# oppo-us-research/PoP-Net

Measured on AMD Instinct MI355X. Metric: depth-frames/sec end-to-end (480x640), higher is better.
Workload: dtype bf16

## Files before the change

popnet_amd/csrc/api.hip:

```cpp
#pragma clang fp contract(off)
#include <cmath>
#include <cstdio>
#include <cstdlib>
#include <cstring>
#include "pn_internal.h"
#include "preproc_pixel.h"

template <typename TIN>
__global__ void preprocess_kernel(const TIN *__restrict__ depth, float *__restrict__ out, int B, int H, int W, int S,
                                  double scale_x, double scale_y, float dmax, float mean, float stdv) {
    const unsigned pix = blockIdx.x * blockDim.x + threadIdx.x;
    if (pix >= (unsigned)(S * S)) return;
    const int b = blockIdx.y;
    const int dy = (int)(pix / (unsigned)S);
    const int dx = (int)(pix - (unsigned)dy * (unsigned)S);
    const size_t gid = (size_t)b * S * S + pix;

    out[gid] = pn_preproc_pixel(depth + (size_t)b * H * W, H, W, dy, dx, scale_x, scale_y, dmax, mean, stdv);
}

PnSwitches pn_read_switches() {
    auto set = [](const char *name) { return getenv(name) != nullptr; };
    auto num = [](const char *name, int unset) { const char *e = getenv(name); return e ? atoi(e) : unset; };
    auto is = [](const char *name, const char *value) { const char *e = getenv(name); return e && !strcmp(e, value); };
    PnSwitches s;
    s.no_conv3 = set("POPNET_NO_CONV3");
    s.conv3_rpg8 = set("POPNET_CONV3_RPG8");
    s.conv3_pt14 = num("POPNET_CONV3_PT14", 0);
    s.conv3_nbuf2 = set("POPNET_CONV3_NBUF2");
    s.generic_c64_off = num("POPNET_GENERIC_C64", 1) == 0;
    if (set("POPNET_CONV4")) s.conv4 = num("POPNET_CONV4", 0) == 0 ? 0 : 1;
    s.no_mix = set("POPNET_NO_MIX");
    s.no_bblock = set("POPNET_NO_BBLOCK");
    s.bblock_x3 = num("POPNET_BBLOCK_X3", 0) != 0;
    s.bb64_static = set("POPNET_BB64_STATIC");
    s.bb64_halves = num("POPNET_BB64_HALVES", 1) == 2 ? 2 : 1;
    s.no_tailfuse = set("POPNET_NO_TAILFUSE");
    s.no_poolfuse = set("POPNET_NO_POOLFUSE");
    s.no_stempool = set("POPNET_NO_STEMPOOL");
    s.no_embed3 = set("POPNET_NO_EMBED3");
    s.train_x3_wide = set("POPNET_TRAIN_X3_WIDE");
    s.train_wgrad_novec = set("POPNET_TRAIN_WGRAD_NOVEC");
    s.trainx_one_stream = num("POPNET_TRAINX_STREAMS", 0) == 1;
    s.trainx_stem_handover = set("POPNET_TRAINX_STEM_HANDOVER");
    s.trainx_stem_gather = is("POPNET_TRAINX_STEM_FWD", "gather");
    s.trainx_stem_bn_separate = is("POPNET_TRAINX_STEM_BN", "separate");
    s.trainx_stem_depth = num("POPNET_TRAINX_STEM_DEPTH", 2);
    s.trainx_pack_gather = is("POPNET_TRAINX_PACK", "gather");
    s.trainx_legacy_wgrad = is("POPNET_TRAINX_WGRAD", "legacy");
    return s;
}

extern "C" {

int pn_abi_version(void) { return PN_ABI_VERSION; }
int pn_build_experiments(void) { return 0; }

pn_ctx *pn_create(int device_id) {
    pn_ctx *ctx = new pn_ctx();
    ctx->device = device_id;
    int ndev = 0;
    hipError_t e = hipGetDeviceCount(&ndev);
    if (e != hipSuccess || device_id < 0 || device_id >= ndev) {
        char buf[256];
        snprintf(buf, sizeof buf, "pn_create: device %d not available (%d devices, %s)", device_id, ndev,
                 hipGetErrorString(e));
        ctx->err = buf;
        ctx->device = -1;
        return ctx;
    }
    hipDeviceProp_t prop;
    if (hipGetDeviceProperties(&prop, device_id) == hipSuccess) ctx->num_cus = prop.multiProcessorCount;
    return ctx;
}

void pn_destroy(pn_ctx *ctx) {
    if (!ctx) return;
    if (ctx->parse_ws) (void)hipFree(ctx->parse_ws);
    pn_parse_big_free(ctx);
    if (ctx->train_ws) (void)hipFree(ctx->train_ws);
    for (void *p : ctx->train_ws_retired) (void)hipFree(p);
    for (auto &e : ctx->train_packs) (void)hipFree(e.buf);
    if (ctx->train_pack_table) (void)hipFree(ctx->train_pack_table);
    delete ctx;
}

int pn_last_error(pn_ctx *ctx, char *buf, size_t buf_len) {
    if (!ctx) return 0;
    if (buf && buf_len) {
        size_t n = ctx->err.size() < buf_len - 1 ? ctx->err.size() : buf_len - 1;
        memcpy(buf, ctx->err.data(), n);
        buf[n] = 0;
    }
    return (int)ctx->err.size();
}

int pn_preprocess(pn_ctx *ctx, const void *depth_dev, int depth_dtype, int B, int H, int W, float *out_dev, int S,
                  float depth_max, float depth_mean, float depth_std, void *hip_stream) {
    if (!ctx) return PN_ERR_INVALID;
    if (ctx->device < 0) return pn_set_error(ctx, PN_ERR_STATE, "context has no device");
    if (!depth_dev || !out_dev || B < 1 || H < 2 || W < 2 || S < 1)
        return pn_set_error(ctx, PN_ERR_INVALID, "pn_preprocess: bad arguments");
    if (W == 2 * S && H == 2 * S)
        return pn_set_error(ctx, PN_ERR_UNSUPPORTED, "pn_preprocess: %dx%d -> %d is an exact 2x decimation, where cv2.resize(INTER_LINEAR) runs INTER_AREA instead: not built", W, H, S);
    const double inv_x = (double)S / (double)W, inv_y = (double)S / (double)H;
    const double scale_x = 1.0 / inv_x, scale_y = 1.0 / inv_y;
    if (B > 65535 || (size_t)S * S > 0x7fffffffu) return pn_set_error(ctx, PN_ERR_INVALID, "pn_preprocess: batch or output size out of range");
    dim3 grid((unsigned)(((size_t)S * S + 255) / 256), (unsigned)B), block(256);
    hipStream_t s = (hipStream_t)hip_stream;
    if (depth_dtype == PN_DEPTH_F16)
        hipLaunchKernelGGL(preprocess_kernel<_Float16>, grid, block, 0, s, (const _Float16 *)depth_dev, out_dev, B, H, W, S,
                           scale_x, scale_y, depth_max, depth_mean, depth_std);
    else if (depth_dtype == PN_DEPTH_F32)
        hipLaunchKernelGGL(preprocess_kernel<float>, grid, block, 0, s, (const float *)depth_dev, out_dev, B, H, W, S,
// ... 26 lines not shown
```

popnet_amd/csrc/conv4_kernel.h:

```cpp
#pragma once
#include "conv3_kernel.h"

#define PN4_ASLOT 8192
constexpr int PN4_RING = 3;
constexpr int PN4_PITCH = 32;
#define PN4_ARING (PN4_RING * PN4_ASLOT)
#define PN4_BQUART (5 * PN4_PITCH * 32 + 1024)
#define PN4_BSTRIP (2 * PN4_BQUART)
#define PN4_BBUF (2 * PN4_BSTRIP)
#define PN4_LDS (PN4_ARING + 2 * PN4_BBUF)

__device__ __forceinline__ void conv4_body(const ConvProblem &P, const int block_x) {
    typedef __bf16 T;
    constexpr int KS = 3, KK = 9, PT = 7, CT = 4, PITCH = PN4_PITCH;
    extern __shared__ __attribute__((aligned(16))) char smem[];

    if (block_x >= P.nblocks) return;
    int bx;
    {
        const int nb = P.nblocks, xcd = block_x & 7, idx = block_x >> 3;
        const int qq = nb >> 3, rr = nb & 7;
        bx = (xcd < rr ? xcd * (qq + 1) : rr * (qq + 1) + (xcd - rr) * qq) + idx;
    }
    const int tid = threadIdx.x;
    const int lane = tid & 63;
    const int wave = __builtin_amdgcn_readfirstlane(tid >> 6);
    const int wp = wave >> 1, wc = wave & 1;
    const int c = lane & 15, q = lane >> 4;

    const int cb = bx % P.cout_blocks;
    const int pair = bx / P.cout_blocks;
    const int nstrips = P.B * P.tiles_per_img;
    const int sid_raw = pair * 2 + wp;
    const bool strip_ok = sid_raw < nstrips;
    const int sid = strip_ok ? sid_raw : nstrips - 1;
    const int tile = sid % P.tiles_per_img;
    const int b = sid / P.tiles_per_img;
    const int ty = tile / P.tiles_x, tx = tile - ty * P.tiles_x;
    const int oy0 = ty * P.R, ox0 = tx * P.Wt;
    const int R = min(P.R, P.Ho - oy0);
    const int Wo = P.Wo;
    const int Wc = min(P.Wt, Wo - ox0);
    const int npix = R * Wc;
    const int HC = Wc + KS - 1;
    const int iy0 = oy0 - 1, ix0 = ox0 - 1;
    const float inv_wc = 1.0f / (float)Wc;
    const int nchunks = P.cin_chunks;

    const char *aptr = (const char *)P.wpack + ((size_t)cb * (size_t)(P.ksteps + 3) * 8 + 2 * wave) * 1024;
    const unsigned alane16 = (unsigned)lane * 16u;
    auto dma_a = [&](int slot) {
        const unsigned dst = (unsigned)(slot * PN4_ASLOT) + (unsigned)__builtin_amdgcn_readfirstlane(wave * 2048);
        pn_glds16_s<0>(aptr, alane16, dst);
        pn_glds16_s<0>(aptr + 1024, alane16, dst + 1024u);
        aptr += PN4_ASLOT;
    };

    const size_t frame_b = ((size_t)b * P.H * P.W * P.in_cs + P.in_coff) * 2;
    const char *img = (const char *)P.in + frame_b;
    const unsigned zero_rel = P.in_zero_off - (unsigned)frame_b;
    unsigned boff[6];
#pragma unroll
    for (int j = 0; j < 6; ++j) {
        const int px = lane >> 1;
        const int iy = iy0 + j, ix = ix0 + px;
        const bool inb = px < HC && (unsigned)ix < (unsigned)P.W && (unsigned)iy < (unsigned)P.H;
        boff[j] = inb ? (unsigned)((iy * P.W + ix) * P.in_cs * 2 + wc * 32 + (lane & 1) * 16) : zero_rel;
    }
    const int nhalves = nchunks * 2, wrap_h = P.in_wrap * 2;
    auto dma_b = [&](int j, int buf, int hh) {
        const unsigned dst = (unsigned)(PN4_ARING + buf * PN4_BBUF + j * (PITCH * 32)) +
                             (unsigned)__builtin_amdgcn_readfirstlane(wp * PN4_BSTRIP + wc * PN4_BQUART);
        const int hs = hh < nhalves ? (hh >= wrap_h ? hh - wrap_h : hh) : 0;
        pn_glds16_s<0>(img + (size_t)hs * 64, boff[j], dst);
    };

#pragma unroll
    for (int j = 0; j < 6; ++j) dma_b(j, 0, 0);
    dma_a(0); dma_a(1); dma_a(2);

    int baddr[PT];
#pragma unroll
    for (int pt = 0; pt < PT; ++pt) {
        const int slot = pt * 16 + c;
        const int s = slot < npix ? slot : 0;
        const int ry = (int)(((float)s + 0.5f) * inv_wc);
        const int rx = s - ry * Wc;
        baddr[pt] = PN4_ARING + wp * PN4_BSTRIP + (q >> 1) * PN4_BQUART + (q & 1) * 16 + (ry * PITCH + rx) * 32;
    }
    const int aaddr = wc * 4096 + lane * 16;
    f32x4 acc[CT][PT];
#pragma unroll
    for (int ct = 0; ct < CT; ++ct)
#pragma unroll
        for (int pt = 0; pt < PT; ++pt) acc[ct][pt] = f32x4{0.f, 0.f, 0.f, 0.f};

    const bool active = (cb * 2 + wc) * 64 < P.cout;

    asm volatile("s_waitcnt vmcnt(0)\n\ts_barrier" ::: "memory");

#define PN4_BOFF(j) (((((j) / PT) / KK) & 1) * PN4_BBUF + (((((j) / PT) % KK) / KS) * PITCH + ((((j) / PT) % KK) % KS)) * 32)
    constexpr int BQ = 6;
    static_assert((2 * KK * PT) % BQ == 0, "queue slot of an item must not depend on the chunk");
    bf16x8 aq[2][CT], bq[BQ];
    if (active) {
#pragma unroll
        for (int ct = 0; ct < CT; ++ct) aq[0][ct] = *reinterpret_cast<const bf16x8 *>(smem + aaddr + ct * 1024);
#pragma unroll
        for (int j = 0; j < BQ - 1; ++j) bq[j] = *reinterpret_cast<const bf16x8 *>(smem + baddr[j % PT] + PN4_BOFF(j));
    }
    asm volatile("s_waitcnt lgkmcnt(0)\n\ts_barrier" ::: "memory");

    auto kloop = [&](auto mathc) {
        constexpr bool MATH = decltype(mathc)::value;
        for (int chunk = 0; chunk < nchunks; ++chunk) {
#pragma clang loop unroll(full)
            for (int ph = 0; ph < 2 * KK; ++ph) {
                const int tap = ph % KK, half = ph / KK;
                const int hh = chunk * 2 + half;
                const int anext = aaddr + ((ph + 1) % 3) * PN4_ASLOT;
                if (tap < 6) dma_b(tap, (half + 1) & 1, hh + 1);
                dma_a(ph % 3);
                if (MATH) {
                    __builtin_amdgcn_sched_barrier(0);
#pragma clang loop unroll(full)
                    for (int pt = 0; pt < PT; ++pt) {
                        const int j = ph * PT + pt, jr = j + BQ - 1;
                        if (pt < CT)
                            aq[(ph + 1) & 1][pt] = *reinterpret_cast<const bf16x8 *>(smem + anext + pt * 1024);
                        bq[jr % BQ] = *reinterpret_cast<const bf16x8 *>(smem + baddr[jr % PT] + PN4_BOFF(jr % (2 * KK * PT)));
#pragma unroll
                        for (int ct = 0; ct < CT; ++ct)
                            acc[ct][pt] = __builtin_amdgcn_mfma_f32_16x16x32_bf16(aq[ph & 1][ct], bq[j % BQ], acc[ct][pt], 0, 0, 0);
                        if (pt < CT) __builtin_amdgcn_sched_group_barrier(0x100, 2, 0);
                        else __builtin_amdgcn_sched_group_barrier(0x100, 1, 0);
                        __builtin_amdgcn_sched_group_barrier(0x008, CT, 0);
                    }
                    __builtin_amdgcn_sched_barrier(0);
                }
                if (tap < 6) asm volatile("s_waitcnt vmcnt(3) lgkmcnt(0)\n\ts_barrier" ::: "memory");
                else asm volatile("s_waitcnt vmcnt(2) lgkmcnt(0)\n\ts_barrier" ::: "memory");
            }
        }
    };
    if (active) kloop(std::true_type{});
    else kloop(std::false_type{});
#undef PN4_BOFF
    asm volatile("s_waitcnt vmcnt(0)" ::: "memory");
    if (!active || !strip_ok) return;

    constexpr int LC = CT * 4;
    const int wave_c0 = (cb * 2 + wc) * 64;
    const int cw = wave_c0 + LC * q;
    const int cout = P.cout, act = P.act;
    float bias[LC];
#pragma unroll
    for (int ct = 0; ct < CT; ++ct) {
        const f32x4 b4 = *reinterpret_cast<const PN_GLOBAL f32x4 *>((const PN_GLOBAL float *)P.bias + cw + 4 * ct);
        bias[4 * ct + 0] = b4[0]; bias[4 * ct + 1] = b4[1]; bias[4 * ct + 2] = b4[2]; bias[4 * ct + 3] = b4[3];
    }
    const int res_cs = P.res_cs, out_cs = P.out_cs, Ho = P.Ho;
    const int split = P.split, res_split = P.res_split;
    const unsigned pix0 = (unsigned)((b * Ho + oy0) * Wo + ox0);
    const bool full = wave_c0 + 64 <= cout && P.out && !P.out_nchw;
    if (full) {
        PN_GLOBAL T *ob = (PN_GLOBAL T *)P.out + P.out_coff + cw;
        const PN_GLOBAL T *rb = P.res ? (const PN_GLOBAL T *)P.res + P.res_coff + cw : nullptr;
        auto finish = [&](auto actc, auto resc) {
            constexpr int ACT = decltype(actc)::value;
            constexpr bool RES = decltype(resc)::value;
#pragma clang loop unroll(full)
            for (int pt = 0; pt < PT; ++pt) {
                const int slot = pt * 16 + c;
                const unsigned t = (unsigned)(baddr[pt] - PN4_ARING - wp * PN4_BSTRIP - (q >> 1) * PN4_BQUART) >> 5;
                const unsigned opix = PITCH == 32 ? pix0 + (t >> 5) * (unsigned)Wo + (t & 31u) : pix0 + (t / (unsigned)PITCH) * (unsigned)Wo + (t % (unsigned)PITCH);
                float v[LC];
#pragma unroll
                for (int ct = 0; ct < CT; ++ct)
#pragma unroll
                    for (int i = 0; i < 4; ++i) v[4 * ct + i] = acc[ct][pt][i] + bias[4 * ct + i];
                if (RES) {
                    for (int pl = 0; pl < (res_split ? 2 : 1); ++pl) {
                        T rv[LC];
                        const PN_GLOBAL u32x4 *rp = reinterpret_cast<const PN_GLOBAL u32x4 *>(rb + (opix * (unsigned)res_cs + (unsigned)(pl * res_split)));
                        reinterpret_cast<u32x4 *>(rv)[0] = rp[0];
                        reinterpret_cast<u32x4 *>(rv)[1] = rp[1];
#pragma unroll
                        for (int k = 0; k < LC; ++k) v[k] += (float)rv[k];
                    }
                }
#pragma unroll
                for (int k = 0; k < LC; ++k) {
                    if (ACT == PN_ACT_RELU) v[k] = v[k] > 0.f ? v[k] : 0.f;
                    else if (ACT == PN_ACT_LEAKY) v[k] = v[k] > 0.f ? v[k] : v[k] * 0.1f;
                    else if (ACT != PN_ACT_NONE) v[k] = pn_activate(v[k], act, cw + k, P.yolo_naf);
                }
                for (int pl = 0; pl < (split ? 2 : 1); ++pl) {
                    T ov[LC];
#pragma unroll
                    for (int k = 0; k < LC; ++k) {
                        const T hi = (T)v[k];
                        ov[k] = pl == 1 ? (T)(v[k] - (float)hi) : hi;
                    }
                    if (slot < npix) {
                        PN_GLOBAL u32x4 *op = reinterpret_cast<PN_GLOBAL u32x4 *>(ob + (opix * (unsigned)out_cs + (unsigned)(pl * split)));
                        op[0] = reinterpret_cast<u32x4 *>(ov)[0];
                        op[1] = reinterpret_cast<u32x4 *>(ov)[1];
                    }
                }
            }
        };
        if (P.res) {
            if (act == PN_ACT_RELU) finish(std::integral_constant<int, PN_ACT_RELU>{}, std::true_type{});
            else if (act == PN_ACT_LEAKY) finish(std::integral_constant<int, PN_ACT_LEAKY>{}, std::true_type{});
            else if (act == PN_ACT_NONE) finish(std::integral_constant<int, PN_ACT_NONE>{}, std::true_type{});
            else finish(std::integral_constant<int, -1>{}, std::true_type{});
        } else {
            if (act == PN_ACT_RELU) finish(std::integral_constant<int, PN_ACT_RELU>{}, std::false_type{});
            else if (act == PN_ACT_LEAKY) finish(std::integral_constant<int, PN_ACT_LEAKY>{}, std::false_type{});
            else if (act == PN_ACT_NONE) finish(std::integral_constant<int, PN_ACT_NONE>{}, std::false_type{});
            else finish(std::integral_constant<int, -1>{}, std::false_type{});
        }
        return;
    }
    {
        const PN_GLOBAL T *res_base = P.res ? (const PN_GLOBAL T *)P.res + P.res_coff + cw : nullptr;
        PN_GLOBAL T *out_base = P.out ? (PN_GLOBAL T *)P.out + P.out_coff + cw : nullptr;
        PN_GLOBAL float *nchw = (PN_GLOBAL float *)P.out_nchw;
#pragma clang loop unroll(full)
        for (int pt = 0; pt < PT; ++pt) {
            const int slot = pt * 16 + c;
            if (slot >= npix || cw >= cout) continue;
            const int ry = (int)(((float)slot + 0.5f) * inv_wc);
            const int rx = slot - ry * Wc;
            const unsigned opix = pix0 + (unsigned)(ry * Wo + rx);
#pragma unroll
            for (int ct = 0; ct < CT; ++ct)
#pragma unroll
                for (int i = 0; i < 4; ++i) {
                    const int k = 4 * ct + i;
                    if (cw + k >= cout) continue;
                    float v = acc[ct][pt][i] + bias[k];
                    if (res_base) v += (float)res_base[opix * (unsigned)res_cs + k];
                    if (res_base && res_split) v += (float)res_base[opix * (unsigned)res_cs + res_split + k];
                    v = pn_activate(v, act, cw + k, P.yolo_naf);
                    if (out_base) {
                        const T hi = (T)v;
                        out_base[opix * (unsigned)out_cs + k] = hi;
                        if (split) {
                            out_base[opix * (unsigned)out_cs + split + k] = (T)(v - (float)hi);
                        }
                    }
                    if (nchw) nchw[((size_t)b * cout + cw + k) * ((size_t)Ho * Wo) + (size_t)(oy0 + ry) * Wo + (ox0 + rx)] = v;
                }
        }
    }
}

__global__ __launch_bounds__(256, 2) void conv4_kernel(const ConvProblem *__restrict__ probs) {
    conv4_body(probs[blockIdx.y], (int)blockIdx.x);
}

static int conv4_launch(pn_ctx *ctx, const ConvLaunch &L, hipStream_t stream) {
    const size_t lds = PN4_LDS;
    static PnLdsAttr attr;
    if (int rc = pn_lds_attr(ctx, attr, reinterpret_cast<const void *>(conv4_kernel), lds)) return rc;
    hipLaunchKernelGGL(conv4_kernel, dim3(L.max_blocks, L.nprob), dim3(256), lds, stream, L.probs_dev);
    PN_HIP_CHECK(ctx, hipGetLastError());
    return PN_OK;
}
```

popnet_amd/csrc/net.hip:

```cpp
#include <cmath>
#include <cstdarg>
#include <cstdio>
#include <algorithm>
#include <cstdlib>
#include <cstring>
#include <map>
#include <memory>
#include <vector>
#include "pn_internal.h"
#include "conv_plan.h"
#include "preproc_pixel.h"

namespace {

struct HostTensor {
    std::vector<int64_t> shape;
    std::vector<float> data;
    size_t numel() const { return data.size(); }
};

struct Buf {
    void *p = nullptr;
    int H = 0, W = 0, C = 0;
    int plane = 0;
// ... 692 lines not shown
    int A1 = new_buf(n, H2, W2, 64);
    int X0 = new_buf(n, H4, W4, 64), X1 = new_buf(n, H4, W4, 64), XT = new_buf(n, H4, W4, 64);
    int Y0 = new_buf(n, H8, W8, 128), Y1 = new_buf(n, H8, W8, 128), YT = new_buf(n, H8, W8, 128), YD = new_buf(n, H8, W8, 128);
    int Na = new_buf(n, H8, W8, 256), Nb = new_buf(n, H8, W8, 256);
    int Ha = new_buf(n, H16, W16, 256), Hb = new_buf(n, H16, W16, 256), Hc = new_buf(n, H16, W16, 128);

    if (int rc = add_stem(n, A1)) return rc;
    std::vector<std::vector<int>> levels;
    auto level = [&](std::vector<int> ids) { levels.push_back(ids); };
    if (n->prec == PN_PREC_BF16 && !n->x3 && n->input_dim == 1 && !n->sw.no_stempool) n->steps.back().stem_pool_buf = X0;
    else levels.push_back({-1, 1, A1, X0, 64, 0});
    int cur = X0, other = X1;
    for (int i = 0; i < 3; ++i) {
        std::string p = "model0.layer1." + std::to_string(i);
        level({add_conv(n, p + ".conv1", p + ".bn1", 3, 1, cur, 0, XT, 0, PN_ACT_RELU)});
        level({add_conv(n, p + ".conv2", p + ".bn2", 3, 1, XT, 0, other, 0, PN_ACT_RELU, cur)});
        std::swap(cur, other);
    }
    {
        const bool embed = n->prec == PN_PREC_BF16 && !n->sw.no_embed3;
        const int c1 = add_conv(n, "model0.layer2.0.conv1", "model0.layer2.0.bn1", 3, 2, cur, 0, YT, 0, PN_ACT_RELU);
        const int cd = add_conv(n, "model0.layer2.0.downsample.0", "model0.layer2.0.downsample.1", embed ? 3 : 1, 2, cur, 0, YD, 0, PN_ACT_NONE);
        n->convs[cd].embed3 = embed;
        level({c1, cd});
    }
    level({add_conv(n, "model0.layer2.0.conv2", "model0.layer2.0.bn2", 3, 1, YT, 0, Y0, 0, PN_ACT_RELU, YD)});
    int yc = Y0, yo = Y1;
    for (int i = 1; i < 4; ++i) {
        std::string p = "model0.layer2." + std::to_string(i);
        level({add_conv(n, p + ".conv1", p + ".bn1", 3, 1, yc, 0, YT, 0, PN_ACT_RELU)});
        level({add_conv(n, p + ".conv2", p + ".bn2", 3, 1, YT, 0, yo, 0, PN_ACT_RELU, yc)});
        std::swap(yc, yo);
    }
    n->named["feat"] = {yc, {0, 128}};
    level({add_conv(n, "model1.0", "model1.1", 3, 1, yc, 0, Na, 0, PN_ACT_LEAKY)});
    level({add_conv(n, "model1.3", "model1.4", 3, 1, Na, 0, Nb, 0, PN_ACT_LEAKY)});
    level({add_conv(n, "model1.6", "model1.7", 3, 1, Nb, 0, Na, 0, PN_ACT_LEAKY)});
    level({add_conv(n, "model1.9", "model1.10", 3, 1, Na, 0, Nb, 0, PN_ACT_LEAKY)});
    level({add_conv(n, "model1.12", "", 3, 1, Nb, 0, Na, 0, PN_ACT_NONE)});
    level({add_conv(n, "model2_1.0", "model2_1.1", 3, 1, Na, 0, Nb, 0, PN_ACT_LEAKY)});
    levels.push_back({-1, 2, Nb, Ha, 256, 0});
    level({add_conv(n, "model2_2.0", "model2_2.1", 3, 1, Ha, 0, Hb, 0, PN_ACT_LEAKY)});
    level({add_conv(n, "model2_3.0", "model2_3.1", 3, 1, Hb, 0, Hc, 0, PN_ACT_LEAKY)});
    level({add_conv(n, "model2_4.0", "", 3, 1, Hc, 0, -1, 0, PN_ACT_YOLO, -1, 3)});

    for (auto &cs : n->convs)
        if (int rc = prepare_conv(n, cs)) return rc;
    for (auto &cs : n->convs) n->flops_per_frame += cs.flops;
    fuse_basic_blocks(n, levels);
    for (auto &lv : levels) {
        if (lv[0] == -1) add_pool(n, lv[1], lv[2], lv[3], lv[4], lv[5]);
        else if (lv[0] == -2) { if (int rc = add_bblock(n, lv[1], lv[2])) return rc; }
        else add_conv_level(n, lv);
    }
    return PN_OK;
}

int refresh_problems(pn_net *n, int B, hipStream_t stream) {
    for (auto &st : n->steps) {
        if (st.type != Step::CONV) continue;
        const ConvSpec &c0 = n->convs[st.conv_ids[0]];
        const int BC = c0.kern == 4 ? 128 : (c0.kern == 3 ? c0.wc * 32 : pn_cfg_couts(c0.cfg));
        st.host_probs.clear();
        int max_blocks = 0;
        bool two_bufs = false, has_tail = false, pool_tail = false;
        for (int id : st.conv_ids) {
            const ConvSpec &cs = n->convs[id];
            const Buf &ib = n->bufs[cs.in_buf];
            ConvProblem P;
            memset(&P, 0, sizeof P);
            const size_t es = n->esize();
            (void)es;
            P.in = ib.p;
            P.wpack = cs.wpack;
            P.bias = cs.bias;
            P.B = B; P.H = ib.H; P.W = ib.W;
            P.Ho = (ib.H + 2 * (cs.ks / 2) - cs.ks) / cs.stride + 1;
            P.Wo = (ib.W + 2 * (cs.ks / 2) - cs.ks) / cs.stride + 1;
            P.cin_chunks = cs.cin_chunks;
            P.in_cs = ib.C; P.in_coff = cs.in_coff;
            if (n->x3 && ib.plane % 64)
                return pn_set_error(n->ctx, PN_ERR_UNSUPPORTED, "bf16x3: input plane of %d channels is not a multiple of 64 (the K loop wraps to the hi plane per 64-channel chunk)", ib.plane);
            P.in_wrap = n->x3 ? 2 * (ib.plane / 64) : (1 << 20);
            P.cout = cs.cout;
            if (cs.out_buf >= 0) { P.out = n->bufs[cs.out_buf].p; P.out_cs = n->bufs[cs.out_buf].C; P.out_coff = cs.out_coff; P.split = n->x3 ? n->bufs[cs.out_buf].plane : 0; }
            if (cs.res_buf >= 0) { P.res = n->bufs[cs.res_buf].p; P.res_cs = n->bufs[cs.res_buf].C; P.res_coff = cs.res_coff; P.res_split = n->x3 ? n->bufs[cs.res_buf].plane : 0; }
            if (cs.nchw_slot >= 0) P.out_nchw = n->nchw_ptr[cs.nchw_slot];
            P.act = cs.act;
            P.yolo_naf = 5 + 3 * n->num_parts;
            P.R = cs.R;
            P.Wt = cs.Wt;
            P.tiles_x = (P.Wo + cs.Wt - 1) / cs.Wt;
            P.tiles_per_img = ((P.Ho + cs.R - 1) / cs.R) * P.tiles_x;
            P.cout_blocks = (cs.cout + BC - 1) / BC;
            P.nblocks = B * P.tiles_per_img * P.cout_blocks;
            if (cs.kern == 4) P.nblocks = ((B * P.tiles_per_img + 1) / 2) * P.cout_blocks;
            P.ksteps = cs.cin_chunks * cs.ks * cs.ks * 2;
            P.ks = cs.ks;
            P.lds_buf_bytes = (int)pn_conv_lds_bytes(n->prec, cs.ks, cs.stride, cs.pitch, cs.R);
            P.lds_two = (cs.cin_chunks > 1 && 2 * (size_t)P.lds_buf_bytes <= 160 * 1024) ? 1 : 0;
            P.in_zero_off = (unsigned)((size_t)n->max_batch * ib.H * ib.W * ib.C * es);
            if (cs.pool_tail) {
                const Buf &pb = n->bufs[cs.pool_out_buf];
                P.tiles_x = (pb.W + 6) / 7;
                P.tiles_per_img = ((pb.H + 2) / 3) * P.tiles_x;
                P.nblocks = B * P.tiles_per_img * P.cout_blocks;
                P.tail_out = pb.p; P.tail_out_cs = pb.C; P.tail_out_coff = cs.pool_out_coff;
                P.tail_split = n->x3 ? pb.plane : 0;
                P.out = nullptr;
                pool_tail = true;
            }
            if (cs.tail_conv >= 0) {
                const ConvSpec &tb = n->convs[cs.tail_conv];
                P.tail_w = cs.tail_wpack; P.tail_bias = cs.tail_bias; P.tail_cout = tb.cout; P.tail_act = tb.act;
                if (tb.out_buf >= 0) { P.tail_out = n->bufs[tb.out_buf].p; P.tail_out_cs = n->bufs[tb.out_buf].C; P.tail_out_coff = tb.out_coff; }
                if (tb.nchw_slot >= 0) P.tail_nchw = n->nchw_ptr[tb.nchw_slot];
                P.out = nullptr;
                has_tail = true;
            }
            if (P.lds_two) two_bufs = true;
            max_blocks = std::max(max_blocks, P.nblocks);
            st.host_probs.push_back(P);
        }
        st.launch.prec = n->prec;
        st.launch.ks = c0.ks; st.launch.stride = c0.stride; st.launch.pitch = c0.pitch; st.launch.cfg = c0.cfg;
        st.launch.nprob = (int)st.host_probs.size();
        st.launch.max_blocks = max_blocks;
        st.launch.lds_bytes = pn_conv_lds_bytes(n->prec, c0.ks, c0.stride, c0.pitch, c0.R) * (two_bufs ? 2 : 1);
        st.launch.kern = c0.kern; st.launch.wc = c0.wc; st.launch.wp = c0.wp; st.launch.nbuf = c0.nbuf; st.launch.pt = c0.pt; st.launch.rpg = c0.rpg;
        if (c0.kern == 3) st.launch.lds_bytes = pn_conv3_lds_bytes(c0.ks, c0.wp, c0.nbuf, c0.rpg);
        st.launch.tail = (c0.kern == 3 && has_tail) ? 1 : (c0.kern == 3 && pool_tail) ? 2 : 0;
        st.launch.mix = 0;
        if (c0.kern == 3) {
            for (int id : st.conv_ids) {
                const ConvSpec &cs = n->convs[id];
                if (cs.ks != c0.ks || (cs.tail_conv >= 0) != (c0.tail_conv >= 0)) st.launch.mix = 1;
                st.launch.lds_bytes = std::max(st.launch.lds_bytes, pn_conv3_lds_bytes(cs.ks, cs.wp, cs.nbuf, cs.rpg));
            }
            if (st.launch.tail == 1) st.launch.lds_bytes = std::max<size_t>(st.launch.lds_bytes, 4 * 7 * 1024 + 1024);
            if (st.launch.tail == 2 && n->x3) st.launch.lds_bytes = std::max<size_t>(st.launch.lds_bytes, 2 * 4 * 7 * 1024);
        }
        if (c0.kern == 4) st.launch.lds_bytes = 0;
        st.launch.probs_dev = st.dev_probs;
        PN_HIP_CHECK(n->ctx, hipMemcpyAsync(st.dev_probs, st.host_probs.data(), st.host_probs.size() * sizeof(ConvProblem),
                                            hipMemcpyHostToDevice, stream));
    }
    n->last_B = B;
    for (int i = 0; i < 4; ++i) n->last_nchw[i] = n->nchw_ptr[i];
    return PN_OK;
}

std::string step_label(const pn_net *n, const Step &st) {
    if (st.type == Step::STEM) {
        if (st.stem_pool_buf >= 0) return "stem7x7_pool_kernel";
        if (st.stem_cin > 1) return "conv2d_forward+nchw_relu_to_nhwc_kernel";
        if (n->prec == PN_PREC_F32) return "stem7x7_kernel";
        return n->x3 ? "stem7x7_mfma_kernel<x3>" : "stem7x7_mfma_kernel";
    }
    if (st.type == Step::POOL) return pn_pool_kernel_label(st.mode, n->x3);
    if (st.type == Step::BBLOCK) return n->x3 ? "bb64x3_kernel" : "bb64_kernel";
    const ConvSpec &c0 = n->convs[st.conv_ids[0]];
    bool mix = false;
    for (int id : st.conv_ids) {
        const ConvSpec &cs = n->convs[id];
        if (cs.ks != c0.ks || (cs.tail_conv >= 0) != (c0.tail_conv >= 0)) mix = true;
    }
// ... 384 lines not shown
```

popnet_amd/csrc/pn_internal.h:

```cpp
#pragma once
#include <hip/hip_runtime.h>
#include <stdint.h>
#include <string>
#include <vector>
#include "../../include/popnet_hip.h"

struct pn_ctx {
    int device = 0;
    std::string err;
    int num_cus = 256;
    void *parse_ws = nullptr;
    size_t parse_ws_bytes = 0;
    bool parse_ws_fixed = false;
    void *parse_big = nullptr;
    void *train_ws = nullptr;
    size_t train_ws_bytes = 0;
    bool train_ws_keep = false;
    std::vector<void *> train_ws_retired;
    bool train_lds_attr = false;
    bool train_x3 = false;
    struct PackEntry { const float *w; int Cout, Cin, flip, x3; void *buf; size_t bytes; bool fresh; };
    bool train_pack_cache = false;
    std::vector<PackEntry> train_packs;
    void *train_pack_table = nullptr;
    size_t train_pack_table_entries = 0;
    size_t train_pack_table_cap = 0;
    unsigned train_pack_blocks = 0;
};

struct PnSwitches {
    bool no_conv3 = false;
    bool conv3_rpg8 = false;
    int conv3_pt14 = 0;
    bool conv3_nbuf2 = false;
    bool generic_c64_off = false;
    int conv4 = -1;
    bool no_mix = false;
    bool no_bblock = false;
    bool bblock_x3 = false;
    bool bb64_static = false;
    int bb64_halves = 1;
    bool no_tailfuse = false;
    bool no_poolfuse = false;
    bool no_stempool = false;
    bool no_embed3 = false;
    bool train_x3_wide = false;
    bool train_wgrad_novec = false;
    bool trainx_one_stream = false;
    bool trainx_stem_handover = false;
    bool trainx_stem_gather = false;
    bool trainx_stem_bn_separate = false;
    int trainx_stem_depth = 2;
    bool trainx_pack_gather = false;
    bool trainx_legacy_wgrad = false;
};
PnSwitches pn_read_switches();

int pn_set_error(pn_ctx *ctx, int code, const char *fmt, ...);
void pn_parse_big_free(pn_ctx *ctx);
int pn_train_ws(pn_ctx *ctx, size_t bytes, void **out);

#define PN_HIP_CHECK(ctx, expr)                                                              \
    do {                                                                                     \
        hipError_t _e = (expr);                                                              \
        if (_e != hipSuccess)                                                                \
            return pn_set_error((ctx), PN_ERR_HIP, "%s failed: %s (%s:%d)", #expr,           \
                                hipGetErrorString(_e), __FILE__, __LINE__);                  \
    } while (0)

struct PnLdsAttr { size_t bytes[64] = {}; };
inline int pn_lds_attr(pn_ctx *ctx, PnLdsAttr &st, const void *kern, size_t bytes) {
    const int d = ctx->device >= 0 && ctx->device < 64 ? ctx->device : 0;
    if (st.bytes[d] >= bytes) return PN_OK;
    PN_HIP_CHECK(ctx, hipFuncSetAttribute(kern, hipFuncAttributeMaxDynamicSharedMemorySize, (int)bytes));
    st.bytes[d] = bytes;
    return PN_OK;
}

enum pn_act {
    PN_ACT_NONE = 0,
    PN_ACT_RELU = 1,
    PN_ACT_LEAKY = 2,
    PN_ACT_SIG_PM2 = 3,
    PN_ACT_SIG = 4,
    PN_ACT_YOLO = 5
};

struct ConvProblem {
    const void *in;
    const void *wpack;
    const float *bias;
    const void *res;
    void *out;
    float *out_nchw;
    int B, H, W;
    int Ho, Wo;
    int cin_chunks;
    int in_cs, in_coff;
    int cout;
    int out_cs, out_coff;
    int res_cs, res_coff;
    int act;
    int yolo_naf;
    int R;
    int Wt, tiles_x;
    int tiles_per_img;
    int cout_blocks;
    int nblocks;
    int ksteps;
    int ks;
    int lds_buf_bytes;
    int lds_two;
    unsigned in_zero_off;
    int split;
    int res_split;
    int in_wrap;
    const void *tail_w;
    const float *tail_bias;
    void *tail_out;
    float *tail_nchw;
    int tail_cout, tail_act, tail_out_cs, tail_out_coff;
    int tail_split;
};

enum pn_conv_cfg {
    PN_CFG_C128 = 0,
    PN_CFG_C64 = 1,
    PN_CFG_C32 = 2,
    PN_CFG_C16 = 3,
    PN_CFG_C64W = 4
};
int pn_cfg_couts(int cfg);
inline int pn_cfg_ct(int cfg) { return cfg == PN_CFG_C16 ? 1 : 2; }
inline int pn_conv_row_channel(int tile, int row, int CT) {
    return (tile / CT) * CT * 16 + 4 * CT * (row >> 2) + 4 * (tile % CT) + (row & 3);
}
int pn_cfg_pixels(int cfg);

struct ConvLaunch {
    int prec;
    int ks;
    int stride;
    int pitch;
    int cfg;
    int kern = 0, wc = 0, wp = 0, nbuf = 0, pt = 7, rpg = 4;
    int tail = 0;
    int mix = 0;
    int nprob;
    int max_blocks;
    size_t lds_bytes;
    const ConvProblem *probs_dev;
};
int pn_launch_conv(pn_ctx *ctx, const ConvLaunch &L, hipStream_t stream);
inline std::string pn_conv_kernel_label(int prec, int kern, bool mix, int ks, int stride, int pitch, int cfg, int wc, int wp, int nbuf, int pt, int rpg) {
    char lb[96];
    if (kern == 4) snprintf(lb, sizeof lb, "conv4_kernel");
    else if (kern == 3 && mix) snprintf(lb, sizeof lb, "conv3_mix_kernel");
    else if (kern == 3) snprintf(lb, sizeof lb, "conv3_kernel<%d, %d, %d, %d, %d, %d>", ks, wc, wp, nbuf, pt, rpg);
    else snprintf(lb, sizeof lb, "conv_mfma_kernel<%d, %d, %d, %d, %d>", prec, ks, stride, pitch, cfg);
    return lb;
}
inline std::string pn_pool_kernel_label(int mode, bool split) {
    char lb[48];
    snprintf(lb, sizeof lb, "pool_kernel<%d%s>", mode, split ? ", split" : "");
    return lb;
}
int pn_launch_conv3(pn_ctx *ctx, const ConvLaunch &L, hipStream_t stream);
int pn_launch_conv4(pn_ctx *ctx, const ConvLaunch &L, hipStream_t stream);

struct BBProblem {
    const void *in;
    void *out;
    const void *wpack;
    const float *bias1, *bias2;
    int B, H, W;
    int in_cs, in_coff, out_cs, out_coff;
    int Wt, tiles_x, tiles_per_img, ntiles;
    unsigned in_zero_off;
    int in_split, out_split;
    int *tickets;
    int halves;
};
int pn_launch_bb64(pn_ctx *ctx, const BBProblem &P, hipStream_t stream);
int pn_launch_bb64x3(pn_ctx *ctx, const BBProblem &P, hipStream_t stream);
size_t pn_conv3_lds_bytes(int ks, int WP, int nbuf, int rpg = 4);
size_t pn_conv_lds_bytes(int prec, int ks, int stride, int pitch, int R);
int pn_conv_stage_maxpx(int prec, int ks, int stride, int pitch, int cfg);

struct PnFrameSrc;
int pn_launch_stem_pool(pn_ctx *ctx, const float *x, const void *wfrag, const float *bias, void *out, int B, int H, int W, int Ho, int Wo,
                        int out_cs, hipStream_t stream, const PnFrameSrc *src);
struct PnFrameSrc;
int pn_launch_stem(pn_ctx *ctx, int prec, const float *x, const float *w, const void *wfrag, const float *bias,
                   void *out, int B, int H, int W, int Ho, int Wo, int out_cs, int split, hipStream_t stream, const PnFrameSrc *src = nullptr);

int pn_launch_pool(pn_ctx *ctx, int prec, int mode, const void *in, void *out, int B, int H, int W,
                   int C, int in_cs, int out_cs, int out_coff, int in_split, int out_split, hipStream_t stream);

// ... 13 lines not shown
```

popnet_amd/csrc/trainx.hip:

```cpp
#include <algorithm>
#include <cstdarg>
#include <cstdio>
#include <cstring>
#include <functional>
#include <map>
#include <string>
#include <vector>
#include "pn_internal.h"
#include "conv_plan.h"
#include "trainx_kernels.h"
#include "trainx_wgrad.h"

namespace {

using tx::bf;

struct TxTensor {
    char *p = nullptr;
    int H = 0, W = 0, plane = 0;
    bool f32 = false;
    int cs() const { return f32 ? plane : 2 * plane; }
    int split() const { return f32 ? 0 : plane; }
    char *at(int ch) const { return p + (size_t)ch * (f32 ? 4 : 2); }
};
// ... 183 lines not shown
    d.first_group = t->pack_groups; d.ngroups = (unsigned)real_groups;
    t->pack_groups += (unsigned)real_groups;
    d.first_unit = t->pack_units; d.nunits = (unsigned)((size_t)pc.cout_pad * pc.kplane / 8);
    t->pack_units += d.nunits;
    t->packs.push_back(d);
    *dst_out = slot;
    return PN_OK;
}

int add_conv_group(pn_trainer *t, const std::vector<ConvUse> &uses) {
    pn_ctx *ctx = t->ctx;
    std::vector<PlannedConv> pcs;
    bool k4 = false, wide[4] = {false, false, false, false};
    long blocks = 0;
    for (const ConvUse &u : uses) {
        const TxLayer &L = t->layers[u.layer];
        const TxTensor &in = t->T[u.in];
        const int rows = u.dgrad ? t->T[L.x].plane : L.cout;
        if (L.ks == 3 && rows >= 64) {
            k4 = true;
            const long strips = (long)t->B * ((in.H + 3) / 4) * ((in.W + 29) / 30);
            blocks += ((strips + 1) / 2) * ((rows + 127) / 128);
        }
        if (rows > 64) wide[L.ks] = true;
    }
    if (blocks < 448) k4 = false;
    for (const ConvUse &u : uses) {
        const TxLayer &L = t->layers[u.layer];
        const TxTensor &in = t->T[u.in];
        PlannedConv pc;
        pc.u = u;
        pc.ks = L.ks;
        pc.rows = u.dgrad ? t->T[L.x].plane : L.cout;
        pc.kplane = in.plane;
        if (pc.kplane % 64) return pn_set_error(ctx, PN_ERR_UNSUPPORTED, "pn_trainer: %s: input plane %d is not a multiple of 64", L.name.c_str(), pc.kplane);
        pc.cin_chunks = (t->f32 ? 1 : 3) * pc.kplane / 64;
        pc.g = ConvGeom();
        const int wc_min = (wide[L.ks] && pc.rows > 32) ? 4 : 0;
        const int prec = t->f32 ? PN_PREC_F32 : PN_PREC_BF16;
        pn_plan_conv_kernel(prec, t->B, ctx->num_cus, in.H, in.W, pc.rows, L.ks, 1, pc.cin_chunks, wc_min, 0, k4 ? 1 : 0, t->sw, pc.g);
        const char *why = "";
        if (int rc = pn_plan_conv_tiles(prec, in.H, in.W, L.ks, 1, pc.g, &why)) return pn_set_error(ctx, rc, "pn_trainer: %s: %s", L.name.c_str(), why);
        if (pc.g.kern == 0 && L.ks == 1 && pc.g.pitch == 16) pc.g.pitch = 32;
        pc.BC = pc.g.kern == 4 ? 128 : (pc.g.kern == 3 ? pc.g.wc * 32 : pn_cfg_couts(pc.g.cfg));
        pc.cout_pad = (pc.rows + pc.BC - 1) / pc.BC * pc.BC;
        pcs.push_back(pc);
    }
    std::vector<bool> used(pcs.size(), false);
    for (size_t i = 0; i < pcs.size(); ++i) {
        if (used[i]) continue;
        std::vector<size_t> members;
        const PlannedConv &a = pcs[i];
        for (size_t j = i; j < pcs.size(); ++j) {
            const PlannedConv &b = pcs[j];
            if (used[j]) continue;
            const bool same = b.ks == a.ks && b.g.pitch == a.g.pitch && b.g.R == a.g.R && b.g.Wt == a.g.Wt && b.g.kern == a.g.kern &&
                              (a.g.kern == 4 || (a.g.kern == 3 ? (b.g.wc == a.g.wc && b.g.wp == a.g.wp && b.g.nbuf == a.g.nbuf && b.g.pt == a.g.pt && b.g.rpg == a.g.rpg) : b.g.cfg == a.g.cfg));
            if (same) { members.push_back(j); used[j] = true; }
        }
        std::vector<ConvProblem> probs;
        int max_blocks = 0;
        bool two_bufs = false;
        for (size_t m : members) {
            const PlannedConv &pc = pcs[m];
            TxLayer &L = t->layers[pc.u.layer];
            const TxTensor &in = t->T[pc.u.in];
            ConvProblem P;
            memset(&P, 0, sizeof P);
            bf *pack = nullptr;
            if (int rc = ensure_pack(t, pc, &pack)) return rc;
            P.in = in.p; P.wpack = pack;
            if (!pc.u.dgrad && L.b) {
                if (!L.bias_pad) {
                    if (int rc = tx_alloc(t, (void **)&L.bias_pad, (size_t)pad64(std::max(pc.cout_pad, 128)) * 4, true)) return rc;
                    tx::BiasDesc bd;
                    bd.src = L.b; bd.dst = L.bias_pad; bd.n = L.cout; bd.npad = pad64(std::max(pc.cout_pad, 128));
                    t->biases.push_back(bd);
                }
                P.bias = L.bias_pad;
            } else P.bias = t->zero_bias;
            P.B = t->B; P.H = in.H; P.W = in.W; P.Ho = in.H; P.Wo = in.W;
            P.cin_chunks = pc.cin_chunks; P.in_cs = in.cs(); P.in_coff = 0;
            P.in_wrap = t->f32 ? (1 << 20) : 2 * (in.plane / 64);
            P.cout = pc.rows;
            if (pc.u.out >= 0) { const TxTensor &o = t->T[pc.u.out]; P.out = o.p; P.out_cs = o.cs(); P.out_coff = pc.u.out_coff; P.split = o.split(); }
            if (pc.u.res >= 0) { const TxTensor &r = t->T[pc.u.res]; P.res = r.p; P.res_cs = r.cs(); P.res_coff = 0; P.res_split = r.split(); }
            P.out_nchw = pc.u.out_nchw;
            P.act = pc.u.act;
            P.yolo_naf = 50;
            P.R = pc.g.R; P.Wt = pc.g.Wt;
            P.tiles_x = (P.Wo + pc.g.Wt - 1) / pc.g.Wt;
            P.tiles_per_img = ((P.Ho + pc.g.R - 1) / pc.g.R) * P.tiles_x;
            P.cout_blocks = (pc.rows + pc.BC - 1) / pc.BC;
            P.nblocks = t->B * P.tiles_per_img * P.cout_blocks;
            if (pc.g.kern == 4) P.nblocks = ((t->B * P.tiles_per_img + 1) / 2) * P.cout_blocks;
            P.ksteps = pc.cin_chunks * pc.ks * pc.ks * 2;
            P.ks = pc.ks;
            P.lds_buf_bytes = (int)pn_conv_lds_bytes(t->f32 ? PN_PREC_F32 : PN_PREC_BF16, pc.ks, 1, pc.g.pitch, pc.g.R);
            P.lds_two = (pc.cin_chunks > 1 && 2 * (size_t)P.lds_buf_bytes <= 160 * 1024) ? 1 : 0;
            P.in_zero_off = (unsigned)((size_t)t->B * in.H * in.W * in.plane * 4);
            if (P.lds_two) two_bufs = true;
            max_blocks = std::max(max_blocks, P.nblocks);
            probs.push_back(P);
            t->flops_conv += 2.0 * (t->f32 ? 1.0 : 3.0) * (double)t->B * in.H * in.W * pc.rows * pc.kplane * pc.ks * pc.ks;
        }
        ConvProblem *dev = nullptr;
        if (int rc = tx_alloc(t, (void **)&dev, probs.size() * sizeof(ConvProblem), false)) return rc;
        PN_HIP_CHECK(ctx, hipMemcpy(dev, probs.data(), probs.size() * sizeof(ConvProblem), hipMemcpyHostToDevice));
        ConvLaunch cl;
        cl.prec = t->f32 ? PN_PREC_F32 : PN_PREC_BF16; cl.ks = a.ks; cl.stride = 1; cl.pitch = a.g.pitch; cl.cfg = a.g.cfg;
        cl.kern = a.g.kern; cl.wc = a.g.wc; cl.wp = a.g.wp; cl.nbuf = a.g.nbuf; cl.pt = a.g.pt; cl.rpg = a.g.rpg;
        cl.tail = 0; cl.mix = 0;
        cl.nprob = (int)probs.size(); cl.max_blocks = max_blocks;
        cl.lds_bytes = pn_conv_lds_bytes(cl.prec, a.ks, 1, a.g.pitch, a.g.R) * (two_bufs ? 2 : 1);
        if (a.g.kern == 3) cl.lds_bytes = pn_conv3_lds_bytes(a.ks, a.g.wp, a.g.nbuf, a.g.rpg);
        if (a.g.kern == 4) cl.lds_bytes = 0;
        cl.probs_dev = dev;
        t->launches.push_back(cl);
        const size_t li = t->launches.size() - 1;
        t->ops.push_back([t, li](hipStream_t s) { return pn_launch_conv(t->ctx, t->launches[li], s); });
        std::string body = jf("\"kernels\": [\"%s\"], \"problems\": [", pn_conv_kernel_label(cl.prec, cl.kern, false, cl.ks, 1, cl.pitch, cl.cfg, cl.wc, cl.wp, cl.nbuf, cl.pt, cl.rpg).c_str());
        for (size_t m = 0; m < members.size(); ++m) {
            const PlannedConv &pc = pcs[members[m]];
            const TxLayer &L = t->layers[pc.u.layer];
            int hs = -1, hb = -1;
            for (int st = 0; st < 2; ++st)
                for (int b = 0; b < 3; ++b)
                    if (pc.u.out_nchw && pc.u.out_nchw == t->head_out[st][b]) { hs = st; hb = b; }
            body += jf("%s{\"layer\": \"%s\", \"dgrad\": %d, \"act\": %d, \"bias\": %d, \"ks\": %d, \"cin\": %d, \"cout\": %d, \"cat\": %d, \"rows\": %d, \"R\": %d, \"Wt\": %d, ",
                       m ? ", " : "", L.name.c_str(), pc.u.dgrad ? 1 : 0, pc.u.act, (!pc.u.dgrad && L.b) ? 1 : 0, pc.ks, L.cin, L.cout, L.cat ? 1 : 0, pc.rows, pc.g.R, pc.g.Wt);
            body += "\"in\": " + jref(pc.u.in, 0, t->T[pc.u.in].plane) + ", \"out\": " + jref(pc.u.out, pc.u.out_coff, pc.rows) + ", \"res\": " + jref(pc.u.res, 0, pc.rows);
            body += hs >= 0 ? jf(", \"nchw\": \"head_out.%d.%d\"}", hs, hb) : std::string(", \"nchw\": null}");
        }
        describe(t, "conv", body + "]");
    }
    return PN_OK;
}

int red_blocks(const pn_trainer *t, long npix, int C, int *ppb) {
    const int PL = 256 / (C / 8);
    long per = std::max<long>((npix + 4 * t->ctx->num_cus - 1) / (4 * t->ctx->num_cus), 8L * PL);
    per = (per + PL - 1) / PL * PL;
    *ppb = (int)per;
    return (int)((npix + per - 1) / per);
}

int need_partial(pn_trainer *t, size_t doubles) { t->partial_doubles = std::max(t->partial_doubles, doubles); return PN_OK; }

struct BnUse { int bn, x, res, y, act; };
struct BnBwdUse { int bn, x, dy, y, dx, dres, act; bool has_res; };

void op_bn_fwd(pn_trainer *t, std::vector<BnUse> uses) {
    const int n = (int)uses.size();
    struct Geo { long npix; int C, ppb, nblk; size_t poff; } g[3];
    size_t poff = 0;
    int max_nblk = 0, max_c = 0;
    long max_items = 0;
    for (int i = 0; i < n; ++i) {
        const TxTensor X = t->T[uses[i].x];
        g[i].npix = (long)t->B * X.H * X.W; g[i].C = t->bns[uses[i].bn].C;
        g[i].nblk = red_blocks(t, g[i].npix, g[i].C, &g[i].ppb);
        g[i].poff = poff; poff += (size_t)g[i].nblk * g[i].C * 2;
        max_nblk = std::max(max_nblk, g[i].nblk); max_c = std::max(max_c, g[i].C); max_items = std::max(max_items, g[i].npix * (g[i].C / 8));
    }
    need_partial(t, poff);
    t->ops.push_back([=](hipStream_t s) {
// ... 768 lines not shown
```

Measured before the change: 67160.

## Add CT=2 conv4 variant for narrow-cout layers and packed bf16 epilogue

Templates the conv4 kernel on the number of cout tiles per wave. When an env switch is set and cout is 64 or less, it uses a CT=2 path in which all four waves work instead of half idling, with a deeper B queue and adjusted wait counts. The epilogue is also rewritten to use packed float2 math, bitcast-based bf16 residual unpacking and packed ReLU on bf16 pairs, with a compile-time split flag. The CT=2 path is off by default, but the epilogue rewrite and the runtime branch in the kernel apply to every launch.

```diff
diff --git a/popnet_amd/csrc/api.hip b/popnet_amd/csrc/api.hip
--- a/popnet_amd/csrc/api.hip
+++ b/popnet_amd/csrc/api.hip
@@ -30,6 +30,7 @@
     s.conv3_nbuf2 = set("POPNET_CONV3_NBUF2");
     s.generic_c64_off = num("POPNET_GENERIC_C64", 1) == 0;
     if (set("POPNET_CONV4")) s.conv4 = num("POPNET_CONV4", 0) == 0 ? 0 : 1;
+    s.conv4_ct2 = num("POPNET_CONV4_CT2", 0) != 0;
     s.no_mix = set("POPNET_NO_MIX");
     s.no_bblock = set("POPNET_NO_BBLOCK");
     s.bblock_x3 = num("POPNET_BBLOCK_X3", 0) != 0;
diff --git a/popnet_amd/csrc/conv4_kernel.h b/popnet_amd/csrc/conv4_kernel.h
--- a/popnet_amd/csrc/conv4_kernel.h
+++ b/popnet_amd/csrc/conv4_kernel.h
@@ -10,9 +10,19 @@
 #define PN4_BBUF (2 * PN4_BSTRIP)
 #define PN4_LDS (PN4_ARING + 2 * PN4_BBUF)
 
+typedef __attribute__((ext_vector_type(2))) float pn4_f32x2;
+typedef __attribute__((ext_vector_type(2))) __bf16 pn4_bf16x2;
+typedef __attribute__((ext_vector_type(2))) short pn4_i16x2;
+__device__ __forceinline__ unsigned pn4_relu_pk(unsigned w) {
+    return __builtin_bit_cast(unsigned, __builtin_elementwise_max(__builtin_bit_cast(pn4_i16x2, w), pn4_i16x2{0, 0}));
+}
+
+template <int CT>
 __device__ __forceinline__ void conv4_body(const ConvProblem &P, const int block_x) {
     typedef __bf16 T;
-    constexpr int KS = 3, KK = 9, PT = 7, CT = 4, PITCH = PN4_PITCH;
+    constexpr int KS = 3, KK = 9, PT = 7, PITCH = PN4_PITCH;
+    constexpr int NA = CT / 2;
+    static_assert(CT == 4 || CT == 2, "4 waves x NA tiles = the 2 * CT tiles of a block");
     extern __shared__ __attribute__((aligned(16))) char smem[];
 
     if (block_x >= P.nblocks) return;
@@ -47,12 +57,12 @@
     const float inv_wc = 1.0f / (float)Wc;
     const int nchunks = P.cin_chunks;
 
-    const char *aptr = (const char *)P.wpack + ((size_t)cb * (size_t)(P.ksteps + 3) * 8 + 2 * wave) * 1024;
+    const char *aptr = (const char *)P.wpack + ((size_t)cb * (size_t)(P.ksteps + 3) * 8 + NA * wave) * 1024;
     const unsigned alane16 = (unsigned)lane * 16u;
     auto dma_a = [&](int slot) {
-        const unsigned dst = (unsigned)(slot * PN4_ASLOT) + (unsigned)__builtin_amdgcn_readfirstlane(wave * 2048);
+        const unsigned dst = (unsigned)(slot * PN4_ASLOT) + (unsigned)__builtin_amdgcn_readfirstlane(wave * NA * 1024);
         pn_glds16_s<0>(aptr, alane16, dst);
-        pn_glds16_s<0>(aptr + 1024, alane16, dst + 1024u);
+        if (CT == 4) pn_glds16_s<0>(aptr + 1024, alane16, dst + 1024u);
         aptr += PN4_ASLOT;
     };
 
@@ -88,20 +98,21 @@
         const int rx = s - ry * Wc;
         baddr[pt] = PN4_ARING + wp * PN4_BSTRIP + (q >> 1) * PN4_BQUART + (q & 1) * 16 + (ry * PITCH + rx) * 32;
     }
-    const int aaddr = wc * 4096 + lane * 16;
+    const int aaddr = wc * CT * 1024 + lane * 16;
     f32x4 acc[CT][PT];
 #pragma unroll
     for (int ct = 0; ct < CT; ++ct)
 #pragma unroll
         for (int pt = 0; pt < PT; ++pt) acc[ct][pt] = f32x4{0.f, 0.f, 0.f, 0.f};
 
-    const bool active = (cb * 2 + wc) * 64 < P.cout;
+    const bool active = CT == 2 || (cb * 2 + wc) * 64 < P.cout;
 
     asm volatile("s_waitcnt vmcnt(0)\n\ts_barrier" ::: "memory");
 
 #define PN4_BOFF(j) (((((j) / PT) / KK) & 1) * PN4_BBUF + (((((j) / PT) % KK) / KS) * PITCH + ((((j) / PT) % KK) % KS)) * 32)
-    constexpr int BQ = 6;
+    constexpr int BQ = CT == 4 ? 6 : 14;
     static_assert((2 * KK * PT) % BQ == 0, "queue slot of an item must not depend on the chunk");
+    static_assert(6 * PT + PT - 1 + BQ - 1 < KK * PT, "phase 6 must not read the next half's image");
     bf16x8 aq[2][CT], bq[BQ];
     if (active) {
 #pragma unroll
@@ -138,20 +149,21 @@
                     }
                     __builtin_amdgcn_sched_barrier(0);
                 }
-                if (tap < 6) asm volatile("s_waitcnt vmcnt(3) lgkmcnt(0)\n\ts_barrier" ::: "memory");
-                else asm volatile("s_waitcnt vmcnt(2) lgkmcnt(0)\n\ts_barrier" ::: "memory");
+                if (tap < 6 && CT == 4) asm volatile("s_waitcnt vmcnt(3) lgkmcnt(0)\n\ts_barrier" ::: "memory");
+                else if (tap < 6 || CT == 4) asm volatile("s_waitcnt vmcnt(2) lgkmcnt(0)\n\ts_barrier" ::: "memory");
+                else asm volatile("s_waitcnt vmcnt(1) lgkmcnt(0)\n\ts_barrier" ::: "memory");
             }
         }
     };
-    if (active) kloop(std::true_type{});
+    if (CT == 2 || active) kloop(std::true_type{});
     else kloop(std::false_type{});
 #undef PN4_BOFF
     asm volatile("s_waitcnt vmcnt(0)" ::: "memory");
     if (!active || !strip_ok) return;
 
-    constexpr int LC = CT * 4;
-    const int wave_c0 = (cb * 2 + wc) * 64;
-    const int cw = wave_c0 + LC * q;
+    constexpr int LC = CT * 4, NQ = CT / 2;
+    const int wave_c0 = CT == 4 ? (cb * 2 + wc) * 64 : cb * 128;
+    const int cw = CT == 4 ? wave_c0 + LC * q : wave_c0 + 16 * q + LC * wc;
     const int cout = P.cout, act = P.act;
     float bias[LC];
 #pragma unroll
@@ -166,60 +178,81 @@
     if (full) {
         PN_GLOBAL T *ob = (PN_GLOBAL T *)P.out + P.out_coff + cw;
         const PN_GLOBAL T *rb = P.res ? (const PN_GLOBAL T *)P.res + P.res_coff + cw : nullptr;
-        auto finish = [&](auto actc, auto resc) {
+        auto finish = [&](auto actc, auto resc, auto splitc) {
             constexpr int ACT = decltype(actc)::value;
-            constexpr bool RES = decltype(resc)::value;
+            constexpr bool RES = decltype(resc)::value, SPLIT = decltype(splitc)::value;
 #pragma clang loop unroll(full)
             for (int pt = 0; pt < PT; ++pt) {
                 const int slot = pt * 16 + c;
                 const unsigned t = (unsigned)(baddr[pt] - PN4_ARING - wp * PN4_BSTRIP - (q >> 1) * PN4_BQUART) >> 5;
                 const unsigned opix = PITCH == 32 ? pix0 + (t >> 5) * (unsigned)Wo + (t & 31u) : pix0 + (t / (unsigned)PITCH) * (unsigned)Wo + (t % (unsigned)PITCH);
-                float v[LC];
-#pragma unroll
-                for (int ct = 0; ct < CT; ++ct)
-#pragma unroll
-                    for (int i = 0; i < 4; ++i) v[4 * ct + i] = acc[ct][pt][i] + bias[4 * ct + i];
+                pn4_f32x2 v[2 * CT];
+#pragma unroll
+                for (int k = 0; k < 2 * CT; ++k)
+                    v[k] = pn4_f32x2{acc[k >> 1][pt][2 * (k & 1)], acc[k >> 1][pt][2 * (k & 1) + 1]} + pn4_f32x2{bias[2 * k], bias[2 * k + 1]};
                 if (RES) {
-                    for (int pl = 0; pl < (res_split ? 2 : 1); ++pl) {
-                        T rv[LC];
+                    for (int pl = 0; pl < (SPLIT && res_split ? 2 : 1); ++pl) {
                         const PN_GLOBAL u32x4 *rp = reinterpret_cast<const PN_GLOBAL u32x4 *>(rb + (opix * (unsigned)res_cs + (unsigned)(pl * res_split)));
-                        reinterpret_cast<u32x4 *>(rv)[0] = rp[0];
-                        reinterpret_cast<u32x4 *>(rv)[1] = rp[1];
-#pragma unroll
-                        for (int k = 0; k < LC; ++k) v[k] += (float)rv[k];
-                    }
-                }
-#pragma unroll
-                for (int k = 0; k < LC; ++k) {
-                    if (ACT == PN_ACT_RELU) v[k] = v[k] > 0.f ? v[k] : 0.f;
-                    else if (ACT == PN_ACT_LEAKY) v[k] = v[k] > 0.f ? v[k] : v[k] * 0.1f;
-                    else if (ACT != PN_ACT_NONE) v[k] = pn_activate(v[k], act, cw + k, P.yolo_naf);
-                }
-                for (int pl = 0; pl < (split ? 2 : 1); ++pl) {
-                    T ov[LC];
-#pragma unroll
-                    for (int k = 0; k < LC; ++k) {
-                        const T hi = (T)v[k];
-                        ov[k] = pl == 1 ? (T)(v[k] - (float)hi) : hi;
+                        u32x4 rr[NQ];
+#pragma unroll
+                        for (int k = 0; k < NQ; ++k) rr[k] = rp[k];
+#pragma unroll
+                        for (int k = 0; k < 2 * CT; ++k) {
+                            const unsigned w = rr[k >> 2][k & 3];
+                            v[k] += pn4_f32x2{__builtin_bit_cast(float, w << 16), __builtin_bit_cast(float, w & 0xffff0000u)};
+                        }
+                    }
+                }
+#pragma unroll
+                for (int k = 0; k < 2 * CT; ++k) {
+                    if (ACT == PN_ACT_LEAKY) {
+                        const pn4_f32x2 m = v[k] * pn4_f32x2{0.1f, 0.1f};
+                        v[k] = pn4_f32x2{__builtin_fmaxf(v[k][0], m[0]), __builtin_fmaxf(v[k][1], m[1])};
+                    } else if (ACT == PN_ACT_RELU) {
+                        if (SPLIT) v[k] = pn4_f32x2{v[k][0] > 0.f ? v[k][0] : 0.f, v[k][1] > 0.f ? v[k][1] : 0.f};
+                    } else if (ACT != PN_ACT_NONE) {
+                        v[k] = pn4_f32x2{pn_activate(v[k][0], act, cw + 2 * k, P.yolo_naf), pn_activate(v[k][1], act, cw + 2 * k + 1, P.yolo_naf)};
+                    }
+                }
+                u32x4 o[NQ];
+#pragma unroll
+                for (int k = 0; k < 2 * CT; ++k) {
+                    const unsigned w = __builtin_bit_cast(unsigned, __builtin_convertvector(v[k], pn4_bf16x2));
+                    o[k >> 2][k & 3] = (ACT == PN_ACT_RELU && !SPLIT) ? pn4_relu_pk(w) : w;
+                }
+                if (slot < npix) {
+                    PN_GLOBAL u32x4 *op = reinterpret_cast<PN_GLOBAL u32x4 *>(ob + opix * (unsigned)out_cs);
+#pragma unroll
+                    for (int k = 0; k < NQ; ++k) op[k] = o[k];
+                }
+                if (SPLIT && split) {
+                    u32x4 o2[NQ];
+#pragma unroll
+                    for (int k = 0; k < 2 * CT; ++k) {
+                        const unsigned w = o[k >> 2][k & 3];
+                        const pn4_f32x2 d = v[k] - pn4_f32x2{__builtin_bit_cast(float, w << 16), __builtin_bit_cast(float, w & 0xffff0000u)};
+                        o2[k >> 2][k & 3] = __builtin_bit_cast(unsigned, __builtin_convertvector(d, pn4_bf16x2));
                     }
                     if (slot < npix) {
-                        PN_GLOBAL u32x4 *op = reinterpret_cast<PN_GLOBAL u32x4 *>(ob + (opix * (unsigned)out_cs + (unsigned)(pl * split)));
-                        op[0] = reinterpret_cast<u32x4 *>(ov)[0];
-                        op[1] = reinterpret_cast<u32x4 *>(ov)[1];
+                        PN_GLOBAL u32x4 *op = reinterpret_cast<PN_GLOBAL u32x4 *>(ob + (opix * (unsigned)out_cs + (unsigned)split));
+#pragma unroll
+                        for (int k = 0; k < NQ; ++k) op[k] = o2[k];
                     }
                 }
             }
         };
-        if (P.res) {
-            if (act == PN_ACT_RELU) finish(std::integral_constant<int, PN_ACT_RELU>{}, std::true_type{});
-            else if (act == PN_ACT_LEAKY) finish(std::integral_constant<int, PN_ACT_LEAKY>{}, std::true_type{});
-            else if (act == PN_ACT_NONE) finish(std::integral_constant<int, PN_ACT_NONE>{}, std::true_type{});
-            else finish(std::integral_constant<int, -1>{}, std::true_type{});
+        auto finish_act = [&](auto resc, auto splitc) {
+            if (act == PN_ACT_RELU) finish(std::integral_constant<int, PN_ACT_RELU>{}, resc, splitc);
+            else if (act == PN_ACT_LEAKY) finish(std::integral_constant<int, PN_ACT_LEAKY>{}, resc, splitc);
+            else if (act == PN_ACT_NONE) finish(std::integral_constant<int, PN_ACT_NONE>{}, resc, splitc);
+            else finish(std::integral_constant<int, -1>{}, resc, splitc);
+        };
+        if (split || res_split) {
+            if (P.res) finish_act(std::true_type{}, std::true_type{});
+            else finish_act(std::false_type{}, std::true_type{});
         } else {
-            if (act == PN_ACT_RELU) finish(std::integral_constant<int, PN_ACT_RELU>{}, std::false_type{});
-            else if (act == PN_ACT_LEAKY) finish(std::integral_constant<int, PN_ACT_LEAKY>{}, std::false_type{});
-            else if (act == PN_ACT_NONE) finish(std::integral_constant<int, PN_ACT_NONE>{}, std::false_type{});
-            else finish(std::integral_constant<int, -1>{}, std::false_type{});
+            if (P.res) finish_act(std::true_type{}, std::false_type{});
+            else finish_act(std::false_type{}, std::false_type{});
         }
         return;
     }
@@ -258,7 +291,9 @@
 }
 
 __global__ __launch_bounds__(256, 2) void conv4_kernel(const ConvProblem *__restrict__ probs) {
-    conv4_body(probs[blockIdx.y], (int)blockIdx.x);
+    const ConvProblem &P = probs[blockIdx.y];
+    if (P.ct2 && P.cout <= 64) conv4_body<2>(P, (int)blockIdx.x);
+    else conv4_body<4>(P, (int)blockIdx.x);
 }
 
 static int conv4_launch(pn_ctx *ctx, const ConvLaunch &L, hipStream_t stream) {
diff --git a/popnet_amd/csrc/net.hip b/popnet_amd/csrc/net.hip
--- a/popnet_amd/csrc/net.hip
+++ b/popnet_amd/csrc/net.hip
@@ -798,6 +798,7 @@
             if (n->x3 && ib.plane % 64)
                 return pn_set_error(n->ctx, PN_ERR_UNSUPPORTED, "bf16x3: input plane of %d channels is not a multiple of 64 (the K loop wraps to the hi plane per 64-channel chunk)", ib.plane);
             P.in_wrap = n->x3 ? 2 * (ib.plane / 64) : (1 << 20);
+            P.ct2 = n->sw.conv4_ct2 ? 1 : 0;
             P.cout = cs.cout;
             if (cs.out_buf >= 0) { P.out = n->bufs[cs.out_buf].p; P.out_cs = n->bufs[cs.out_buf].C; P.out_coff = cs.out_coff; P.split = n->x3 ? n->bufs[cs.out_buf].plane : 0; }
             if (cs.res_buf >= 0) { P.res = n->bufs[cs.res_buf].p; P.res_cs = n->bufs[cs.res_buf].C; P.res_coff = cs.res_coff; P.res_split = n->x3 ? n->bufs[cs.res_buf].plane : 0; }
diff --git a/popnet_amd/csrc/pn_internal.h b/popnet_amd/csrc/pn_internal.h
--- a/popnet_amd/csrc/pn_internal.h
+++ b/popnet_amd/csrc/pn_internal.h
@@ -35,6 +35,7 @@
     bool conv3_nbuf2 = false;
     bool generic_c64_off = false;
     int conv4 = -1;
+    bool conv4_ct2 = false;
     bool no_mix = false;
     bool no_bblock = false;
     bool bblock_x3 = false;
@@ -114,6 +115,7 @@
     unsigned in_zero_off;
     int split;
     int res_split;
+    int ct2;
     int in_wrap;
     const void *tail_w;
     const float *tail_bias;
diff --git a/popnet_amd/csrc/trainx.hip b/popnet_amd/csrc/trainx.hip
--- a/popnet_amd/csrc/trainx.hip
+++ b/popnet_amd/csrc/trainx.hip
@@ -289,6 +289,7 @@
             P.B = t->B; P.H = in.H; P.W = in.W; P.Ho = in.H; P.Wo = in.W;
             P.cin_chunks = pc.cin_chunks; P.in_cs = in.cs(); P.in_coff = 0;
             P.in_wrap = t->f32 ? (1 << 20) : 2 * (in.plane / 64);
+            P.ct2 = t->sw.conv4_ct2 ? 1 : 0;
             P.cout = pc.rows;
             if (pc.u.out >= 0) { const TxTensor &o = t->T[pc.u.out]; P.out = o.p; P.out_cs = o.cs(); P.out_coff = pc.u.out_coff; P.split = o.split(); }
             if (pc.u.res >= 0) { const TxTensor &r = t->T[pc.u.res]; P.res = r.p; P.res_cs = r.cs(); P.res_coff = 0; P.res_split = r.split(); }
```

After: 67220, median of 2. Within noise of the previous version (+0.1%).
